# Audio-WestlakeU/FullSubNet

Measured on NVIDIA H100. Metric: frames_per_sec, higher is better.
Workload: dtype f16x3(hi+lo split, fp32-class)xf32acc

## Files before the change

### fullsubnet_b200/csrc/fsn_subband_tc.cu

```cuda
#include <cuda_fp16.h>
#include <stdlib.h>
#include <string.h>

#include "fsn_internal.cuh"
#include "fsn_tc_ptx.cuh"
#include "fsn_wgmma.cuh"

namespace fsn {
namespace tc {

using namespace ptx;

constexpr int NB = 32;
constexpr int KB = 64;
constexpr int KS = 32;
constexpr int US = 64;
constexpr int W_SUB = US * KS * 2;
constexpr int W_TILE = 4 * W_SUB;
constexpr int S_KBLK = NB * KB * 2;
constexpr int X_BLK = NB * KS * 2;
constexpr int MAX_STAGES = 4;
constexpr int MAX_MT = 3;
constexpr int OUT_T = 8;
constexpr int NTHREADS = 128 + 128 * MAX_MT;

struct PackedLayout {
  int H, MT, nkb0, nkb1, parts;
  size_t tiles0, tiles1;
  size_t off_bias, off_fcw, off_fcb, bytes;
};

__host__ __device__ inline PackedLayout packed_layout(int H, bool x3) {
  PackedLayout L;
  L.H = H; L.MT = H / 128;
  L.nkb0 = 1 + H / KS; L.nkb1 = 2 * H / KS;
  L.parts = x3 ? 2 : 1;
  L.tiles0 = (size_t)L.MT * L.nkb0 * L.parts;
  L.tiles1 = (size_t)L.MT * L.nkb1 * L.parts;
  L.off_bias = 2 * (L.tiles0 + L.tiles1) * W_TILE;
  L.off_fcw = L.off_bias + (size_t)2 * 4 * H * sizeof(float);
  L.off_fcb = L.off_fcw + (size_t)2 * H * sizeof(float);
  L.bytes = L.off_fcb + 256;
  return L;
}

__global__ void pack_kernel(const float* __restrict__ wih0, const float* __restrict__ whh0,
                            const float* __restrict__ wih1, const float* __restrict__ whh1,
                            const float* __restrict__ bih0, const float* __restrict__ bhh0,
                            const float* __restrict__ bih1, const float* __restrict__ bhh1,
                            const float* __restrict__ fcw, const float* __restrict__ fcb, int H, int Ksb, int x3,
                            int fc_out, uint8_t* __restrict__ out) {
  const PackedLayout L = packed_layout(H, x3 != 0);
  const size_t per_half = L.tiles0 + L.tiles1;
  const size_t total = 2 * per_half * 4 * US * 4;
  for (size_t i = blockIdx.x * (size_t)blockDim.x + threadIdx.x; i < total; i += (size_t)gridDim.x * blockDim.x) {
    const int c = (int)(i & 3);
    const int r = (int)((i >> 2) & (US - 1));
    const int g = (int)((i >> 8) & 3);
    const size_t st_abs = i >> 10;
    const int half = (int)(st_abs / per_half);
    size_t st = st_abs - half * per_half;
    const int layer = st >= L.tiles0;
    if (layer) st -= L.tiles0;
    const int part = (int)(st % L.parts);
    st /= L.parts;
    const int nkb = layer ? L.nkb1 : L.nkb0;
    const int kb = (int)(st % nkb);
    const int m = (int)(st / nkb);
    const int wrow = g * H + (half * L.MT + m) * US + r;
    __half v[8];
#pragma unroll
    for (int e = 0; e < 8; ++e) {
      const int kk = c * 8 + e;
      float w = 0.f;
      if (layer == 0) {
        if (kb == 0) { if (kk < Ksb) w = wih0[(size_t)wrow * Ksb + kk]; }
        else w = whh0[(size_t)wrow * H + (kb - 1) * KS + kk];
      } else {
        const int k = kb * KS + kk;
        w = (k < H) ? wih1[(size_t)wrow * H + k] : whh1[(size_t)wrow * H + (k - H)];
      }
      const __half hi = __float2half_rn(w);
      v[e] = part ? __float2half_rn(w - __half2float(hi)) : hi;
    }
    uint8_t* dst = out + st_abs * W_TILE + g * W_SUB + swz64_off(r, c * 8);
    *reinterpret_cast<uint4*>(dst) = *reinterpret_cast<const uint4*>(v);
  }
  float* bias = reinterpret_cast<float*>(out + L.off_bias);
  float* pfcw = reinterpret_cast<float*>(out + L.off_fcw);
  float* pfcb = reinterpret_cast<float*>(out + L.off_fcb);
  for (int i = blockIdx.x * blockDim.x + threadIdx.x; i < 4 * H; i += gridDim.x * blockDim.x) {
    bias[i] = bih0[i] + bhh0[i];
    bias[4 * H + i] = bih1[i] + bhh1[i];
  }
  for (int i = blockIdx.x * blockDim.x + threadIdx.x; i < 2 * H; i += gridDim.x * blockDim.x)
    pfcw[i] = (i < fc_out * H) ? fcw[i] : 0.f;
  if (blockIdx.x == 0 && threadIdx.x < 2) pfcb[threadIdx.x] = ((int)threadIdx.x < fc_out) ? fcb[threadIdx.x] : 0.f;
}

struct Smem {
  uint32_t w, x, h0, h1, lo, fcw, fcp, outst, rows, bars, total;
};
__host__ __device__ inline Smem smem_plan(int H, int stages, bool x3) {
  Smem s;
  const int nkh = H / KB;
  uint32_t o = 0;
  s.w = o; o += stages * W_TILE;
  s.x = o; o += 2 * X_BLK;
  s.h0 = o; o += 2 * nkh * S_KBLK;
  s.h1 = o; o += nkh * S_KBLK;
  s.lo = o; o += x3 ? (o - s.x) : 0;
  s.fcw = o; o += 4 * MAX_MT * 2 * NB * 4;
  s.fcp = o; o += 2 * 2 * NB * 4;
  s.outst = o; o += NB * 2 * OUT_T * 4;
  s.rows = o; o += NB * 16;
  s.bars = o; o += 256;
  s.total = o;
  return s;
}

struct Bars {
  uint64_t w_full[MAX_STAGES], w_empty[MAX_STAGES];
  uint64_t x_full[2], x_empty[2];
  uint64_t h0_ready[2], h0_empty[2];
  uint64_t h1_ready, h1_empty, fc_done;
  uint64_t l1_done;
  uint64_t fcp_full[2], fcp_empty[2];
  uint64_t turn[MAX_MT];
};
static_assert(sizeof(Bars) <= 256, "barrier block too large");

struct RowInfo {
  int src_b, src_f;
  float scale;
  int out_idx;
};

struct KArgs {
  const uint8_t* packed;
  const float* magT; const float* fbT; const float* inv2;
  const float* unit_scale;
  float* crm;
  int R, F, Tp, la, T, Ns, Nf, H, Ksb, act, Fsub, stages, cluster;
  int src_T, shrink;
  RowMap map;
  long long* stamps;
  int stamp_ctas, stamp_its;
};

enum ProbeField {
  PF_T_BEGIN = 0,
  PF_T_MMA0 = 1,
  PF_T_MMA1 = 2,
  PF_T_END = 3,
  PF_OPERAND = 4,
  PF_TURN = 5,
  PF_W_FULL = 6,
  PF_WAIT_GROUP = 7,
  PF_GROUP_LAT = 8,
  PF_STAGES = 9,
  PF_CELL = 10,
  PF_L1_DONE = 11,
  PF_H1_EMPTY = 12,
  PF_H0_EMPTY = 13,
  PF_FC_DONE = 14,
  PF_GT_BEGIN = 15,
  PROBE_FIELDS = 16
};
constexpr int PROBE_SLOTS = MAX_MT + 1;
static_assert(PROBE_FIELDS == FSN_SB_PROBE_FIELDS && PROBE_SLOTS == FSN_SB_PROBE_SLOTS,
              "probe record layout differs from fsn_b200.h (and fullsubnet_b200/_lib.py)");

__device__ __forceinline__ long long globaltimer() {
  uint64_t t;
  asm volatile("mov.u64 %0, %%globaltimer;" : "=l"(t));
  return (long long)t;
}

__device__ __forceinline__ float act_apply(float v, int act) {
  switch (act) {
    case FSN_ACT_RELU: return fmaxf(v, 0.f);
    case FSN_ACT_TANH: return tanhf(v);
    case FSN_ACT_RELU6: return fminf(fmaxf(v, 0.f), 6.f);
    default: return v;
  }
}
template <bool X3> __device__ __forceinline__ float sg(float x) { return X3 ? 1.0f / (1.0f + expf(-x)) : fast_sigmoid(x); }
template <bool X3> __device__ __forceinline__ float th(float x) { return X3 ? 1.0f - 2.0f / (1.0f + expf(2.0f * x)) : fast_tanh(x); }

__device__ __forceinline__ void release_stage(uint32_t bar, uint32_t pred, uint32_t local, uint32_t remote,
                                              uint32_t rank) {
  mbar_arrive_elect_if(bar, pred & local);
  mbar_arrive_remote_elect_if(bar, rank, pred & remote);
}

template <bool X3, bool PROBE>
__global__ void __launch_bounds__(NTHREADS, 1) sb_lstm_tc_kernel(const __grid_constant__ KArgs a) {
  constexpr int PARTS = X3 ? 2 : 1;
  long long pt = 0;
  auto mark = [&]() -> uint32_t {
    if constexpr (PROBE) {
      const long long n = clock64();
      const uint32_t d = (uint32_t)(n - pt);
      pt = n;
      return d;
    } else {
      return 0u;
    }
  };
  auto record = [&](int it, int layer, int slot) -> long long* {
    return a.stamps + ((((size_t)blockIdx.x * a.stamp_its + it) * 2 + layer) * PROBE_SLOTS + slot) * PROBE_FIELDS;
  };
  const bool probe_cta = PROBE && (int)blockIdx.x < a.stamp_ctas;
  extern __shared__ uint8_t smem_raw[];
  uint8_t* smem = smem_raw + ((1024u - (smem_u32(smem_raw) & 1023u)) & 1023u);
  const int H = a.H;
  const int MT = H / 128;
  const int nkh = H / KB;
  const int STAGES = a.stages;
  const int CL = a.cluster;
  const uint32_t cl_rank = cluster_ctarank();
  const int half = (int)(cl_rank & 1u);
  const uint32_t peer = cl_rank ^ 1u;
  const uint16_t cl_mask = (uint16_t)((0x55u & ((1u << (2 * CL)) - 1u)) << half);
  const Smem sp = smem_plan(H, STAGES, X3);
  const uint32_t LO = sp.lo - sp.x;
  const PackedLayout PL = packed_layout(H, X3);
  Bars& bars = *reinterpret_cast<Bars*>(smem + sp.bars);
  RowInfo* rows = reinterpret_cast<RowInfo*>(smem + sp.rows);
  float* fc_part = reinterpret_cast<float*>(smem + sp.fcw);
  float* fcp = reinterpret_cast<float*>(smem + sp.fcp);
  float* outst = reinterpret_cast<float*>(smem + sp.outst);
  const int warp = threadIdx.x >> 5, lane = threadIdx.x & 31;
  const int row0 = (blockIdx.x >> 1) * NB;
  const int Tp = a.Tp;

  if (threadIdx.x == 0) {
    for (int s = 0; s < STAGES; ++s) { mbar_init(&bars.w_full[s], 1); mbar_init(&bars.w_empty[s], CL); }
    for (int i = 0; i < 2; ++i) {
      mbar_init(&bars.x_full[i], 1); mbar_init(&bars.x_empty[i], 4 * MT);
      mbar_init(&bars.h0_ready[i], 5 * MT);
      mbar_init(&bars.h0_empty[i], MT);
      mbar_init(&bars.fcp_full[i], 1); mbar_init(&bars.fcp_empty[i], 1);
    }
    mbar_init(&bars.h1_ready, 5 * MT);
    mbar_init(&bars.h1_empty, MT);
    mbar_init(&bars.fc_done, 1);
    mbar_init(&bars.l1_done, 4 * MT);
    for (int m = 0; m < MAX_MT; ++m) mbar_init(&bars.turn[m], 4);
    asm volatile("fence.mbarrier_init.release.cluster;" ::: "memory");
  }
  if (threadIdx.x < NB) {
    RowInfo ri;
    const int r = row0 + threadIdx.x;
    ri.src_b = -1; ri.src_f = 0; ri.scale = 0.f; ri.out_idx = 0;
    if (r < a.R) {
      row_to_unit(a.map, r, ri.src_b, ri.src_f);
      ri.scale = a.inv2[ri.src_b];
      const int bq = r / a.Fsub, fq = r - bq * a.Fsub;
      ri.out_idx = bq * 2 * a.Fsub + fq;
    }
    rows[threadIdx.x] = ri;
  }
  {
    uint4* z = reinterpret_cast<uint4*>(smem + sp.x);
    const int n16 = (sp.fcw - sp.x) / 16;
    for (int i = threadIdx.x; i < n16; i += blockDim.x) z[i] = make_uint4(0, 0, 0, 0);
  }
  fence_proxy_async_smem();
  __syncthreads();
  cluster_sync_all();

  if (warp < 4) {
    asm volatile("setmaxnreg.dec.sync.aligned.u32 56;");
  if (warp == 0) {
    const uint8_t* stream = a.packed + (size_t)half * (PL.tiles0 + PL.tiles1) * W_TILE;
    uint32_t stage = 0, phase = 0;
    for (int it = 0; it <= Tp; ++it) {
      const size_t t_begin = (it < Tp) ? 0 : PL.tiles0;
      const size_t t_end = (it >= 1) ? PL.tiles0 + PL.tiles1 : PL.tiles0;
      const uint8_t* src = stream + t_begin * W_TILE;
      long long p_t0 = 0, p_g0 = 0;
      uint32_t p_empty = 0;
      if constexpr (PROBE) { p_g0 = globaltimer(); p_t0 = clock64(); pt = p_t0; }
      for (size_t tile = t_begin; tile < t_end; ++tile, src += W_TILE) {
        mark();
        mbar_wait_cta<false>(&bars.w_empty[stage], phase ^ 1);
        p_empty += mark();
        if (elect_one()) {
          mbar_expect_tx(&bars.w_full[stage], W_TILE);
          if (CL == 1) {
            bulk_g2s(smem + sp.w + stage * W_TILE, src, W_TILE, &bars.w_full[stage]);
          } else {
            const uint32_t slice = W_TILE / CL, off = (cl_rank >> 1) * slice;
            bulk_g2s_mc(smem + sp.w + stage * W_TILE + off, src + off, slice, &bars.w_full[stage], cl_mask);
          }
        }
        __syncwarp();
        if (++stage == (uint32_t)STAGES) { stage = 0; phase ^= 1; }
      }
      if (probe_cta && it < a.stamp_its && lane == 0) {
        long long* r = record(it, 0, MAX_MT);
        r[PF_T_BEGIN] = p_t0; r[PF_T_END] = clock64(); r[PF_OPERAND] = p_empty;
        r[PF_STAGES] = (long long)(t_end - t_begin); r[PF_GT_BEGIN] = p_g0;
      }
    }
  } else if (warp == 2) {
    const int nmag = 2 * a.Ns + 1;
    for (int t = 0; t < Tp; ++t) {
      mbar_wait_cta<true>(&bars.x_empty[t & 1], ((t >> 1) & 1) ^ 1);
      uint8_t* xb = smem + sp.x + (t & 1) * X_BLK;
      int f0 = t, f1 = t + 1;
      if (a.shrink > 1 && t > 0) { f0 = 1 + (t - 1) * a.shrink; f1 = min(f0 + a.shrink, a.src_T); }
      const float wmean = 1.0f / (float)(f1 - f0);
#pragma unroll 4
      for (int n = 0; n < NB; ++n) {
        const RowInfo ri = rows[n];
        float v = 0.f;
        if (ri.src_b >= 0 && lane < a.Ksb) {
          const int col = (lane < nmag) ? reflect_idx(ri.src_f + lane - a.Ns, a.F)
                                        : reflect_idx(ri.src_f + (lane - nmag) - a.Nf, a.F);
          const float* src = (lane < nmag) ? a.magT : a.fbT;
          if (a.shrink <= 1) {
            v = src[((size_t)ri.src_b * a.src_T + t) * a.F + col];
            v *= a.unit_scale ? a.unit_scale[(size_t)t * a.R + row0 + n] : ri.scale;
          } else {
            for (int fr = f0; fr < f1; ++fr) v += src[((size_t)ri.src_b * a.src_T + fr) * a.F + col];
            v *= wmean * (a.unit_scale ? a.unit_scale[(size_t)t * a.R + row0 + n] : ri.scale);
          }
        }
        const __half hi = __float2half_rn(v);
        *reinterpret_cast<__half*>(xb + swz64_off(n, lane)) = hi;
        if (X3) *reinterpret_cast<__half*>(xb + LO + swz64_off(n, lane)) = __float2half_rn(v - __half2float(hi));
      }
      fence_proxy_async_smem();
      __syncwarp();
      if (lane == 0) mbar_arrive(&bars.x_full[t & 1]);
    }
  } else if (warp == 3) {
    const float fcb0 = half ? 0.f : reinterpret_cast<const float*>(a.packed + PL.off_fcb)[0];
    const float fcb1 = half ? 0.f : reinterpret_cast<const float*>(a.packed + PL.off_fcb)[1];
    const RowInfo ri = rows[lane];
    int staged = 0, t_stage0 = 0;
    for (int t = 0; t < Tp; ++t) {
      mbar_wait_cta<true>(&bars.h1_ready, t & 1);
      float s0 = fcb0, s1 = fcb1;
      if (t >= a.la) {
        for (int w = 0; w < 4 * MT; ++w) {
          s0 += fc_part[(w * 2 + 0) * NB + lane];
          s1 += fc_part[(w * 2 + 1) * NB + lane];
        }
      }
      __syncwarp();
      if (lane == 0) mbar_arrive(&bars.fc_done);
      if (t < a.la) continue;
      const int u = t - a.la, b = u & 1;
      float* pb = fcp + b * 2 * NB;
      if (half) {
        mbar_wait<true>(&bars.fcp_empty[b], ((u >> 1) & 1) ^ 1);
        st_remote_f32(pb + lane, peer, s0);
        st_remote_f32(pb + NB + lane, peer, s1);
        __syncwarp();
        if (lane == 0) mbar_arrive_cluster(&bars.fcp_full[b], peer);
        continue;
      }
      mbar_wait<true>(&bars.fcp_full[b], (u >> 1) & 1);
      s0 += pb[lane];
      s1 += pb[NB + lane];
      __syncwarp();
      if (lane == 0) mbar_arrive_cluster(&bars.fcp_empty[b], peer);
      if (staged == 0) t_stage0 = u;
      outst[(lane * 2 + 0) * OUT_T + staged] = act_apply(s0, a.act);
      outst[(lane * 2 + 1) * OUT_T + staged] = act_apply(s1, a.act);
      ++staged;
      if (staged == OUT_T || t == Tp - 1) {
        if (ri.src_b >= 0) {
#pragma unroll
          for (int o = 0; o < 2; ++o) {
            float* dst = a.crm + ((size_t)ri.out_idx + (size_t)o * a.Fsub) * a.T + t_stage0;
            for (int i = 0; i < staged; ++i) dst[i] = outst[(lane * 2 + o) * OUT_T + i];
          }
        }
        staged = 0;
      }
    }
  }
  } else {
    asm volatile("setmaxnreg.inc.sync.aligned.u32 152;");
    const int m = __shfl_sync(0xffffffffu, (warp - 4) >> 2, 0);
    const int q = __shfl_sync(0xffffffffu, warp & 3, 0);
    const int s = half * MT + m;
    if (m < MT) {
      const float* bias_g = reinterpret_cast<const float*>(a.packed + PL.off_bias);
      const float* fcw = reinterpret_cast<const float*>(a.packed + PL.off_fcw);
      float* my_part = fc_part + (size_t)(warp - 4) * 2 * NB;
      float c0[16], c1[16];
#pragma unroll
      for (int i = 0; i < 16; ++i) c0[i] = c1[i] = 0.f;
      const uint32_t a_lo0 = wg::desc_lo(smem_u32(smem + sp.w));
      const uint32_t w_full0 = smem_u32(&bars.w_full[0]), w_empty0 = smem_u32(&bars.w_empty[0]);
      const uint32_t turn_next = smem_u32(&bars.turn[m + 1 < MT ? m + 1 : 0]);
      const uint32_t rel_local = CL == 1 && q == 0, rel_remote = CL > 1 && q < CL;
      const uint32_t rel_rank = 2 * q + half;
      int h0_seen = 0, h1_seen = 0, turns = 0;
      bool first_block = true;
      size_t tile_base = 0;
      for (int it = 0; it <= Tp; ++it) {
        for (int layer = 0; layer < 2; ++layer) {
          const int t = it - layer;
          if (t < 0 || t >= Tp) continue;
          long long p_t0 = 0, p_g0 = 0, p_mma0 = 0, p_mma1 = 0, p_commit = 0, p_commit_prev = 0;
          uint32_t p_opnd = 0, p_turn = 0, p_wfull = 0, p_wgw = 0, p_lat = 0, p_cell = 0, p_l1 = 0, p_h1e = 0, p_h0e = 0,
                   p_fc = 0;
          if constexpr (PROBE) { p_g0 = globaltimer(); p_t0 = clock64(); pt = p_t0; }
          if (layer == 0) {
            mbar_wait_cta<false>(&bars.x_full[t & 1], (t >> 1) & 1);
            for (; h0_seen < t; ++h0_seen) mbar_wait_cta<false>(&bars.h0_ready[h0_seen & 1], (h0_seen >> 1) & 1);
          } else {
            for (; h0_seen < t + 1; ++h0_seen) mbar_wait_cta<false>(&bars.h0_ready[h0_seen & 1], (h0_seen >> 1) & 1);
            for (; h1_seen < t; ++h1_seen) mbar_wait_cta<false>(&bars.h1_ready, h1_seen & 1);
          }
          p_opnd += mark();
          const uint32_t x_addr = smem_u32(smem + sp.x + (t & 1) * X_BLK);
          const uint32_t h0_cur = smem_u32(smem + sp.h0 + (t & 1) * nkh * S_KBLK);
          const uint32_t h0_prev = smem_u32(smem + sp.h0 + ((t + 1) & 1) * nkh * S_KBLK);
          const uint32_t h1_prev = smem_u32(smem + sp.h1);
          const int nkb = layer ? PL.nkb1 : PL.nkb0;
          const size_t first = tile_base + (layer ? ((it < Tp) ? PL.tiles0 : 0) : 0) + (size_t)m * nkb * PARTS;
          float acc[4][16];
#pragma unroll
          for (int g = 0; g < 4; ++g) {
#pragma unroll
            for (int i = 0; i < 16; ++i) acc[g][i] = 0.f;
            wg::fence_operand(acc[g]);
          }
          int prev_stage = -1;
          if (m > 0 || !first_block) { mbar_wait_cta<false>(&bars.turn[m], turns & 1); ++turns; }
          first_block = false;
          p_turn += mark();
          p_mma0 = pt;
          int stage = __shfl_sync(0xffffffffu, (int)(first % (size_t)STAGES), 0);
          uint32_t wphase = __shfl_sync(0xffffffffu, (uint32_t)((first / (size_t)STAGES) & 1), 0);
          auto issue_stage = [&](int part, uint32_t bd, uint32_t b_hi, uint32_t ends_block) {
            mark();
            mbar_wait_cta_warp(w_full0 + 8 * stage, wphase);
            p_wfull += mark();
            mbar_arrive_elect_if(turn_next, ends_block);
            wg::fence();
            const uint32_t ad = a_lo0 + stage * (W_TILE >> 4);
#pragma unroll
            for (int kk = 0; kk < 2; ++kk)
#pragma unroll
              for (int g = 0; g < 4; ++g) {
                const uint32_t a_off = g * (W_SUB >> 4) + kk * 2;
                wg::mma_f16_n32_w(acc[g], ad, a_off, wg::DESC_SW64_HI, bd, kk * 2, b_hi);
                if (X3 && part == 0) wg::mma_f16_n32_w(acc[g], ad, a_off, wg::DESC_SW64_HI, bd, (LO >> 4) + kk * 2, b_hi);
              }
            wg::commit();
            if constexpr (PROBE) p_commit = clock64();
            mark();
            wg::wait<1>();
            p_wgw += mark();
            if constexpr (PROBE) {
              if (prev_stage >= 0) p_lat += (uint32_t)(pt - p_commit_prev);
              p_commit_prev = p_commit;
            }
            release_stage(w_empty0 + 8 * prev_stage, prev_stage >= 0, rel_local, rel_remote, rel_rank);
            prev_stage = stage;
            if (++stage == STAGES) { stage = 0; wphase ^= 1; }
          };
          if (layer == 0) {
#pragma unroll
            for (int part = 0; part < PARTS; ++part) issue_stage(part, wg::desc_lo(x_addr), wg::DESC_SW64_HI, 0u);
          }
          const int nseg = layer ? 2 : 1;
          int seg = 0;
          do {
            uint32_t bd = wg::desc_lo(layer == 0 ? h0_prev : seg == 0 ? h0_cur : h1_prev);
            int kb = 0;
            do {
              const uint32_t ends_block = seg == nseg - 1 && kb == nkh - 1;
#pragma unroll
              for (int part = 0; part < PARTS; ++part) issue_stage(part, bd, wg::DESC_SW128_HI, 0u);
#pragma unroll
              for (int part = 0; part < PARTS; ++part)
                issue_stage(part, bd + (64 >> 4), wg::DESC_SW128_HI, part == PARTS - 1 ? ends_block : 0u);
              bd += S_KBLK >> 4;
            } while (++kb < nkh);
          } while (++seg < nseg);
          mark();
          wg::wait<0>();
#pragma unroll
          for (int g = 0; g < 4; ++g) wg::fence_operand(acc[g]);
          p_wgw += mark();
          if constexpr (PROBE) { p_lat += (uint32_t)(pt - p_commit_prev); p_mma1 = pt; }
          release_stage(w_empty0 + 8 * prev_stage, 1u, rel_local, rel_remote, rel_rank);
          if (lane == 0) mbar_arrive(layer ? &bars.l1_done : &bars.x_empty[t & 1]);
          if (layer == 1 && lane == 0) {
            if (q == 2) mbar_arrive_remote(&bars.h0_empty[t & 1], peer);
            if (q == 3) mbar_arrive_remote(&bars.h1_empty, peer);
          }
          p_cell += mark();
          if (layer == 1 && t >= 1) mbar_wait_cta<false>(&bars.fc_done, (t - 1) & 1);
          p_fc += mark();
          float fsum[2][8];
#pragma unroll
          for (int i = 0; i < 16; ++i) fsum[i >> 3][i & 7] = 0.f;
          __half hv[2][8];
          __half lv[2][8];
          uint8_t* hb = smem + (layer ? sp.h1 : sp.h0 + (t & 1) * nkh * S_KBLK) + s * S_KBLK;
#pragma unroll
          for (int hh = 0; hh < 2; ++hh) {
            const int u = s * US + 16 * q + (lane >> 2) + 8 * hh;
            const float* bl = bias_g + (layer ? 4 * H : 0);
            const float bi = bl[u], bff = bl[H + u], bg = bl[2 * H + u], bo = bl[3 * H + u];
            const float w0 = fcw[u], w1 = fcw[H + u];
#pragma unroll
            for (int j = 0; j < 4; ++j)
#pragma unroll
              for (int e = 0; e < 2; ++e) {
                const int ri = 4 * j + 2 * hh + e;
                const int ci = hh * 8 + j * 2 + e;
                const float cp = layer ? c1[ci] : c0[ci];
                const float cn = sg<X3>(acc[1][ri] + bff) * cp + sg<X3>(acc[0][ri] + bi) * th<X3>(acc[2][ri] + bg);
                if (layer) c1[ci] = cn; else c0[ci] = cn;
                const float h = sg<X3>(acc[3][ri] + bo) * th<X3>(cn);
                const __half hi = __float2half_rn(h);
                hv[hh][j * 2 + e] = hi;
                lv[hh][j * 2 + e] = __float2half_rn(h - __half2float(hi));
                if (layer) { fsum[0][j * 2 + e] += h * w0; fsum[1][j * 2 + e] += h * w1; }
              }
          }
          if (layer == 1) {
#pragma unroll
            for (int o = 0; o < 2; ++o)
#pragma unroll
              for (int r = 0; r < 8; ++r) {
                float v = fsum[o][r];
                v += __shfl_xor_sync(0xffffffffu, v, 4);
                v += __shfl_xor_sync(0xffffffffu, v, 8);
                v += __shfl_xor_sync(0xffffffffu, v, 16);
                fsum[o][r] = v;
              }
            if (lane < 4) {
#pragma unroll
              for (int o = 0; o < 2; ++o)
#pragma unroll
                for (int r = 0; r < 8; ++r) my_part[o * NB + 8 * (r >> 1) + 2 * lane + (r & 1)] = fsum[o][r];
            }
            p_cell += mark();
            mbar_wait_cta<false>(&bars.l1_done, t & 1);
            p_l1 += mark();
            mbar_wait_cta<false>(&bars.h1_empty, t & 1);
            p_h1e += mark();
          } else if (t >= 2) {
            p_cell += mark();
            mbar_wait_cta<false>(&bars.h0_empty[t & 1], ((t - 2) >> 1) & 1);
            p_h0e += mark();
          }
#pragma unroll
          for (int hh = 0; hh < 2; ++hh) {
            const int u = 16 * q + (lane >> 2) + 8 * hh;
            uint8_t* ub = hb + (u & 7) * 2;
            const int chunk = u >> 3;
#pragma unroll
            for (int j = 0; j < 4; ++j)
#pragma unroll
              for (int e = 0; e < 2; ++e) {
                const int n = 8 * j + 2 * (lane & 3) + e;
                uint8_t* p = ub + (n >> 3) * 1024 + (n & 7) * 128 + ((chunk ^ (n & 7)) << 4);
                *reinterpret_cast<__half*>(p) = hv[hh][j * 2 + e];
                if (X3) *reinterpret_cast<__half*>(p + LO) = lv[hh][j * 2 + e];
              }
          }
          fence_proxy_async_smem();
          __syncwarp();
          uint64_t* ready = layer ? &bars.h1_ready : &bars.h0_ready[t & 1];
          if (lane == 0) mbar_arrive(ready);
          named_sync(1 + m, 128);
          if (q == 0 && lane == 0) {
            mbar_arrive_expect_tx_remote(ready, peer, PARTS * S_KBLK);
            bulk_s2s_remote(hb, S_KBLK, ready, peer);
            if (X3) bulk_s2s_remote(hb + LO, S_KBLK, ready, peer);
          }
          if constexpr (PROBE) {
            p_cell += mark();
            if (probe_cta && it < a.stamp_its && q == 0 && lane == 0) {
              long long* r = record(it, layer, m);
              r[PF_T_BEGIN] = p_t0; r[PF_T_MMA0] = p_mma0; r[PF_T_MMA1] = p_mma1; r[PF_T_END] = pt;
              r[PF_OPERAND] = p_opnd; r[PF_TURN] = p_turn; r[PF_W_FULL] = p_wfull; r[PF_WAIT_GROUP] = p_wgw;
              r[PF_GROUP_LAT] = p_lat; r[PF_STAGES] = nkb * PARTS; r[PF_CELL] = p_cell; r[PF_L1_DONE] = p_l1;
              r[PF_H1_EMPTY] = p_h1e; r[PF_H0_EMPTY] = p_h0e; r[PF_FC_DONE] = p_fc; r[PF_GT_BEGIN] = p_g0;
            }
          }
        }
        tile_base += ((it < Tp) ? PL.tiles0 : 0) + ((it >= 1) ? PL.tiles1 : 0);
      }
    }
  }

  __syncthreads();
  cluster_sync_all();
}

}

static int sb_ksb(const fsn_model_desc* d) { return (2 * d->sb_num_neighbors + 1) + (2 * d->fb_num_neighbors + 1); }

static bool sb_tc_shape_ok(int H, int Ksb) { return H % 128 == 0 && H / 128 <= tc::MAX_MT && H >= 128 && Ksb <= tc::KS; }

bool sb_tc_supported(const fsn_model_desc* d) {
  if (d->cell_type != FSN_CELL_LSTM) return false;
  return sb_tc_shape_ok(d->sb_hidden, sb_ksb(d));
}

size_t sb_tc_packed_bytes_raw(int H, bool x3) { return tc::packed_layout(H, x3).bytes; }

size_t sb_tc_packed_bytes(const fsn_model_desc* d) {
  if (!sb_tc_supported(d)) return 0;
  return sb_tc_packed_bytes_raw(d->sb_hidden, d->precision == FSN_PREC_F16X3_TC);
}

int sb_tc_pack_raw(const fsn_seq_weights* sb, int H, int Ksb, int fc_out, void* packed, cudaStream_t st, bool x3) {
  FSN_REQUIRE(sb_tc_shape_ok(H, Ksb), FSN_ERR_UNSUPPORTED,
              "the fp16 tensor-core LSTM stack needs a hidden size in {128,256,384} and an input width <= 32");
  int dev = 0, sms = 132;
  cudaGetDevice(&dev);
  cudaDeviceGetAttribute(&sms, cudaDevAttrMultiProcessorCount, dev);
  tc::pack_kernel<<<sms * 4, 256, 0, st>>>(sb->w_ih[0], sb->w_hh[0], sb->w_ih[1], sb->w_hh[1], sb->b_ih[0], sb->b_hh[0],
                                           sb->b_ih[1], sb->b_hh[1], sb->fc_w, sb->fc_b, H, Ksb, x3 ? 1 : 0, fc_out,
                                           (uint8_t*)packed);
  FSN_CHECK_LAUNCH("sb pack_kernel");
  return FSN_OK;
}

int sb_tc_pack(const fsn_model_desc* d, const fsn_seq_weights* sb, void* packed, cudaStream_t st) {
  FSN_REQUIRE(sb_tc_supported(d), FSN_ERR_UNSUPPORTED,
              "FSN_PREC_F16_TC / FSN_PREC_F16X3_TC need sb_hidden in {128,256,384} and sub-band input width <= 32");
  return sb_tc_pack_raw(sb, d->sb_hidden, sb_ksb(d), 2, packed, st, d->precision == FSN_PREC_F16X3_TC);
}

template <bool X3, bool PROBE = false>
static int sb_tc_config(int H, int stages, int cluster, int pairs, cudaStream_t st, cudaLaunchConfig_t& cfg,
                        cudaLaunchAttribute* attr) {
  const tc::Smem sp = tc::smem_plan(H, stages, X3);
  const size_t smem = sp.total + 1024;
  int rc = check_cuda(cudaFuncSetAttribute(tc::sb_lstm_tc_kernel<X3, PROBE>, cudaFuncAttributeMaxDynamicSharedMemorySize,
                                           (int)smem), "sb_lstm_tc smem attr");
  if (rc) return rc;
  memset(&cfg, 0, sizeof(cfg));
  cfg.gridDim = dim3(2 * pairs);
  cfg.blockDim = dim3(128 + 128 * (H / 128));
  cfg.dynamicSmemBytes = smem;
  cfg.stream = st;
  attr[0].id = cudaLaunchAttributeClusterDimension;
  attr[0].val.clusterDim.x = 2 * cluster;
  attr[0].val.clusterDim.y = 1;
  attr[0].val.clusterDim.z = 1;
  cfg.attrs = attr;
  cfg.numAttrs = 1;
  return FSN_OK;
}

template <bool X3, bool PROBE>
static int sb_tc_launch(const tc::KArgs& a, int H, cudaStream_t st) {
  const int pairs = cdiv(cdiv(a.R, tc::NB), a.cluster) * a.cluster;
  cudaLaunchConfig_t cfg;
  cudaLaunchAttribute attr[1];
  int rc = sb_tc_config<X3, PROBE>(H, a.stages, a.cluster, pairs, st, cfg, attr);
  if (rc) return rc;
  rc = check_cuda(cudaLaunchKernelEx(&cfg, tc::sb_lstm_tc_kernel<X3, PROBE>, a), "sb_lstm_tc_kernel launch");
  if (rc) return rc;
  FSN_CHECK_LAUNCH("sb_lstm_tc_kernel");
  return FSN_OK;
}

int sb_tc_forward(const SbTcArgs& s, cudaStream_t st) {
  tc::KArgs a;
  a.packed = (const uint8_t*)s.packed;
  a.magT = s.magT; a.fbT = s.fbT; a.inv2 = s.inv2; a.unit_scale = s.unit_scale; a.crm = s.crm;
  a.R = s.map.B * s.map.Fsub; a.F = s.F; a.Tp = s.steps > 0 ? s.steps : s.Tp; a.la = s.la; a.T = a.Tp - s.la;
  a.src_T = s.Tp; a.shrink = s.shrink > 1 ? s.shrink : 1;
  a.Ns = s.Ns; a.Nf = s.Nf; a.H = s.H; a.Ksb = (2 * s.Ns + 1) + (2 * s.Nf + 1); a.act = s.act;
  a.Fsub = s.map.Fsub; a.map = s.map;
  a.stamps = s.stamps; a.stamp_ctas = s.stamp_ctas; a.stamp_its = s.stamp_its;
  FSN_REQUIRE(sb_tc_shape_ok(a.H, a.Ksb), FSN_ERR_UNSUPPORTED, "sb_lstm_tc: unsupported hidden size %d / input width %d",
              a.H, a.Ksb);
  static int stages_env = -1;
  if (stages_env < 0) {
    const char* e = getenv("FSN_TC_STAGES");
    stages_env = e ? atoi(e) : 4;
    if (stages_env < 2) stages_env = 2;
    if (stages_env > tc::MAX_STAGES) stages_env = tc::MAX_STAGES;
  }
  static int cluster_env = -1;
  if (cluster_env < 0) {
    const char* e = getenv("FSN_TC_CLUSTER");
    cluster_env = e ? atoi(e) : 1;
    if (cluster_env != 1 && cluster_env != 2 && cluster_env != 4) cluster_env = 1;
  }
  a.stages = s.stages ? s.stages : stages_env;
  a.cluster = s.cluster ? s.cluster : cluster_env;
  if (s.stamps) return s.x3 ? sb_tc_launch<true, true>(a, s.H, st) : sb_tc_launch<false, true>(a, s.H, st);
  return s.x3 ? sb_tc_launch<true, false>(a, s.H, st) : sb_tc_launch<false, false>(a, s.H, st);
}

}

extern "C" size_t fsn_debug_sb_lstm_tc_packed_bytes(int H, int x3) {
  return fsn::sb_tc_shape_ok(H, 0) ? fsn::sb_tc_packed_bytes_raw(H, x3 != 0) : 0;
}

extern "C" int fsn_debug_sb_lstm_tc_max_clusters(int H, int x3, int stages, int cluster, int* clusters) {
  using namespace fsn;
  FSN_REQUIRE(cluster == 1 || cluster == 2 || cluster == 4, FSN_ERR_UNSUPPORTED,
              "sb_lstm_tc: cluster size %d (1, 2 or 4)", cluster);
  FSN_REQUIRE(stages >= 2 && stages <= tc::MAX_STAGES, FSN_ERR_UNSUPPORTED, "sb_lstm_tc: ring depth %d (2, 3 or 4)",
              stages);
  FSN_REQUIRE(sb_tc_shape_ok(H, 0), FSN_ERR_UNSUPPORTED, "sb_lstm_tc: unsupported hidden size %d", H);
  FSN_REQUIRE(clusters, FSN_ERR_SHAPE, "sb_lstm_tc: missing output");
  cudaLaunchConfig_t cfg;
  cudaLaunchAttribute attr[1];
  int rc = x3 ? sb_tc_config<true>(H, stages, cluster, cluster, nullptr, cfg, attr)
              : sb_tc_config<false>(H, stages, cluster, cluster, nullptr, cfg, attr);
  if (rc) return rc;
  return x3 ? check_cuda(cudaOccupancyMaxActiveClusters(clusters, tc::sb_lstm_tc_kernel<true, false>, &cfg), "sb_lstm_tc occupancy")
            : check_cuda(cudaOccupancyMaxActiveClusters(clusters, tc::sb_lstm_tc_kernel<false, false>, &cfg), "sb_lstm_tc occupancy");
}

static int sb_lstm_tc_hook(const fsn_seq_weights* sb, int H, int Ns, int Nf, int fc_out, int act, int x3,
                           const float* magT, const float* fbT, int B, int F, int src_T, int G, const float* inv2,
                           const float* unit_scale, int la, int steps, int shrink, int stages, int cluster, void* packed,
                           float* crm, long long* stamps, int stamp_ctas, int stamp_steps, fsn_stream_t stream) {
  using namespace fsn;
  FSN_REQUIRE(cluster == 0 || cluster == 1 || cluster == 2 || cluster == 4, FSN_ERR_UNSUPPORTED,
              "sb_lstm_tc: cluster size %d (0, 1, 2 or 4)", cluster);
  FSN_REQUIRE(stages == 0 || (stages >= 2 && stages <= tc::MAX_STAGES), FSN_ERR_UNSUPPORTED,
              "sb_lstm_tc: ring depth %d (0, 2, 3 or 4)", stages);
  FSN_REQUIRE(sb && magT && fbT && inv2 && packed && crm, FSN_ERR_SHAPE, "sb_lstm_tc: missing buffer");
  FSN_REQUIRE(B > 0 && F > 1 && src_T > 0 && Ns >= 0 && Nf >= 0 && Ns < F && Nf < F, FSN_ERR_SHAPE,
              "sb_lstm_tc: bad shape B=%d F=%d src_T=%d Ns=%d Nf=%d", B, F, src_T, Ns, Nf);
  FSN_REQUIRE(fc_out == 1 || fc_out == 2, FSN_ERR_SHAPE, "sb_lstm_tc: fc_out %d (1 or 2)", fc_out);
  FSN_REQUIRE(act >= FSN_ACT_NONE && act <= FSN_ACT_RELU6, FSN_ERR_SHAPE, "sb_lstm_tc: activation %d", act);
  FSN_REQUIRE(shrink >= 1 && G >= 1, FSN_ERR_SHAPE, "sb_lstm_tc: shrink %d / groups %d", shrink, G);
  const int g = (B > 1 && G > 1) ? G : 1;
  FSN_REQUIRE(B == 1 || B > G, FSN_ERR_SHAPE, "sb_lstm_tc: batch size %d <= num_groups %d", B, G);
  const int Fsub = g > 1 ? F / g : F;
  FSN_REQUIRE(Fsub > 0, FSN_ERR_SHAPE, "sb_lstm_tc: num_freqs < num_groups");
  const int max_steps = shrink > 1 ? 1 + cdiv(src_T - 1, shrink) : src_T;
  FSN_REQUIRE(steps > 0 && steps <= max_steps && la >= 0 && la < steps, FSN_ERR_SHAPE,
              "sb_lstm_tc: steps %d / look-ahead %d for %d source frames (shrink %d)", steps, la, src_T, shrink);
  FSN_REQUIRE(!(unit_scale && shrink > 1), FSN_ERR_UNSUPPORTED, "sb_lstm_tc: per-step scales with time down-sampling");
  FSN_REQUIRE(sb_tc_shape_ok(H, (2 * Ns + 1) + (2 * Nf + 1)), FSN_ERR_UNSUPPORTED,
              "sb_lstm_tc: unsupported hidden size %d / input width %d", H, (2 * Ns + 1) + (2 * Nf + 1));
  if (stamps) {
    const int ctas = 2 * cdiv(B * Fsub, tc::NB);
    FSN_REQUIRE(stamp_ctas >= 1 && stamp_ctas <= ctas, FSN_ERR_SHAPE, "sb_lstm_tc probe: %d sampled CTAs (1 .. %d)",
                stamp_ctas, ctas);
    FSN_REQUIRE(stamp_steps >= 1 && stamp_steps <= steps + 1, FSN_ERR_SHAPE,
                "sb_lstm_tc probe: %d sampled iterations (1 .. steps + 1 = %d)", stamp_steps, steps + 1);
  }
  cudaStream_t st = (cudaStream_t)stream;
  int rc = sb_tc_pack_raw(sb, H, (2 * Ns + 1) + (2 * Nf + 1), fc_out, packed, st, x3 != 0);
  if (rc) return rc;
  SbTcArgs a;
  memset(&a, 0, sizeof(a));
  a.packed = packed; a.magT = magT; a.fbT = fbT; a.inv2 = inv2; a.unit_scale = unit_scale; a.crm = crm;
  a.B = B; a.F = F; a.Tp = src_T; a.la = la; a.Ns = Ns; a.Nf = Nf; a.H = H; a.act = act;
  a.steps = steps; a.shrink = shrink; a.x3 = x3 != 0;
  a.map = RowMap{B, F, Fsub, g};
  a.stages = stages; a.cluster = cluster;
  a.stamps = stamps; a.stamp_ctas = stamp_ctas; a.stamp_its = stamp_steps;
  return sb_tc_forward(a, st);
}

extern "C" int fsn_debug_sb_lstm_tc(const fsn_seq_weights* sb, int H, int Ns, int Nf, int fc_out, int act, int x3,
                                    const float* magT, const float* fbT, int B, int F, int src_T, int G,
                                    const float* inv2, const float* unit_scale, int la, int steps, int shrink, int stages,
                                    int cluster, void* packed, float* crm, fsn_stream_t stream) {
  return sb_lstm_tc_hook(sb, H, Ns, Nf, fc_out, act, x3, magT, fbT, B, F, src_T, G, inv2, unit_scale, la, steps, shrink,
                         stages, cluster, packed, crm, nullptr, 0, 0, stream);
}

extern "C" int fsn_debug_sb_lstm_tc_probe(const fsn_seq_weights* sb, int H, int Ns, int Nf, int fc_out, int act, int x3,
                                          const float* magT, const float* fbT, int B, int F, int src_T, int G,
                                          const float* inv2, const float* unit_scale, int la, int steps, int shrink,
                                          int stages, int cluster, void* packed, float* crm, long long* stamps,
                                          int stamp_ctas, int stamp_steps, fsn_stream_t stream) {
  using namespace fsn;
  FSN_REQUIRE(stamps, FSN_ERR_SHAPE, "sb_lstm_tc probe: missing stamp buffer");
  return sb_lstm_tc_hook(sb, H, Ns, Nf, fc_out, act, x3, magT, fbT, B, F, src_T, G, inv2, unit_scale, la, steps, shrink,
                         stages, cluster, packed, crm, stamps, stamp_ctas, stamp_steps, stream);
}
```

Baseline: 127,500.

## Hand off weight-ring turn early using double-generation full barriers

Duplicates the w_full mbarrier set so consumers can tell apart two consecutive generations of the weight ring. The turn token now passes to the next M-tile warpgroup several K-blocks before the current block finishes, instead of at its last stage. The next consumer can then start waiting on and consuming tiles while the current one drains its tail, hiding handoff latency. The cost is more complex phase tracking, and a parity aliasing risk if the generation assumptions are off.

```diff
diff --git a/fullsubnet_b200/csrc/fsn_subband_tc.cu b/fullsubnet_b200/csrc/fsn_subband_tc.cu
--- a/fullsubnet_b200/csrc/fsn_subband_tc.cu
+++ b/fullsubnet_b200/csrc/fsn_subband_tc.cu
@@ -120,7 +120,7 @@
 }
 
 struct Bars {
-  uint64_t w_full[MAX_STAGES], w_empty[MAX_STAGES];
+  uint64_t w_full[2][MAX_STAGES], w_empty[MAX_STAGES];
   uint64_t x_full[2], x_empty[2];
   uint64_t h0_ready[2], h0_empty[2];
   uint64_t h1_ready, h1_empty, fc_done;
@@ -129,6 +129,7 @@
   uint64_t turn[MAX_MT];
 };
 static_assert(sizeof(Bars) <= 256, "barrier block too large");
+static_assert(1 + 256 / KS >= 2 * MAX_STAGES, "a block of MT >= 2 must span two ring generations (turn[])");
 
 struct RowInfo {
   int src_b, src_f;
@@ -236,7 +237,9 @@
   const int Tp = a.Tp;
 
   if (threadIdx.x == 0) {
-    for (int s = 0; s < STAGES; ++s) { mbar_init(&bars.w_full[s], 1); mbar_init(&bars.w_empty[s], CL); }
+    for (int s = 0; s < STAGES; ++s) {
+      mbar_init(&bars.w_full[0][s], 1); mbar_init(&bars.w_full[1][s], 1); mbar_init(&bars.w_empty[s], CL);
+    }
     for (int i = 0; i < 2; ++i) {
       mbar_init(&bars.x_full[i], 1); mbar_init(&bars.x_empty[i], 4 * MT);
       mbar_init(&bars.h0_ready[i], 5 * MT);
@@ -288,12 +291,13 @@
         mbar_wait_cta<false>(&bars.w_empty[stage], phase ^ 1);
         p_empty += mark();
         if (elect_one()) {
-          mbar_expect_tx(&bars.w_full[stage], W_TILE);
+          uint64_t* full = &bars.w_full[phase][stage];
+          mbar_expect_tx(full, W_TILE);
           if (CL == 1) {
-            bulk_g2s(smem + sp.w + stage * W_TILE, src, W_TILE, &bars.w_full[stage]);
+            bulk_g2s(smem + sp.w + stage * W_TILE, src, W_TILE, full);
           } else {
             const uint32_t slice = W_TILE / CL, off = (cl_rank >> 1) * slice;
-            bulk_g2s_mc(smem + sp.w + stage * W_TILE + off, src + off, slice, &bars.w_full[stage], cl_mask);
+            bulk_g2s_mc(smem + sp.w + stage * W_TILE + off, src + off, slice, full, cl_mask);
           }
         }
         __syncwarp();
@@ -398,8 +402,9 @@
 #pragma unroll
       for (int i = 0; i < 16; ++i) c0[i] = c1[i] = 0.f;
       const uint32_t a_lo0 = wg::desc_lo(smem_u32(smem + sp.w));
-      const uint32_t w_full0 = smem_u32(&bars.w_full[0]), w_empty0 = smem_u32(&bars.w_empty[0]);
+      const uint32_t w_full0 = smem_u32(&bars.w_full[0][0]), w_empty0 = smem_u32(&bars.w_empty[0]);
       const uint32_t turn_next = smem_u32(&bars.turn[m + 1 < MT ? m + 1 : 0]);
+      const int turn_kb = nkh - min(nkh, STAGES / PARTS);
       const uint32_t rel_local = CL == 1 && q == 0, rel_remote = CL > 1 && q < CL;
       const uint32_t rel_rank = 2 * q + half;
       int h0_seen = 0, h1_seen = 0, turns = 0;
@@ -440,12 +445,13 @@
           p_turn += mark();
           p_mma0 = pt;
           int stage = __shfl_sync(0xffffffffu, (int)(first % (size_t)STAGES), 0);
-          uint32_t wphase = __shfl_sync(0xffffffffu, (uint32_t)((first / (size_t)STAGES) & 1), 0);
-          auto issue_stage = [&](int part, uint32_t bd, uint32_t b_hi, uint32_t ends_block) {
+          uint32_t wset = __shfl_sync(0xffffffffu, (uint32_t)((first / (size_t)STAGES) & 1), 0);
+          uint32_t wphase = __shfl_sync(0xffffffffu, (uint32_t)((first / (size_t)STAGES / 2) & 1), 0);
+          auto issue_stage = [&](int part, uint32_t bd, uint32_t b_hi, uint32_t hand_on) {
             mark();
-            mbar_wait_cta_warp(w_full0 + 8 * stage, wphase);
+            mbar_wait_cta_warp(w_full0 + wset * (8 * MAX_STAGES) + 8 * stage, wphase);
             p_wfull += mark();
-            mbar_arrive_elect_if(turn_next, ends_block);
+            mbar_arrive_elect_if(turn_next, hand_on);
             wg::fence();
             const uint32_t ad = a_lo0 + stage * (W_TILE >> 4);
 #pragma unroll
@@ -467,7 +473,7 @@
             }
             release_stage(w_empty0 + 8 * prev_stage, prev_stage >= 0, rel_local, rel_remote, rel_rank);
             prev_stage = stage;
-            if (++stage == STAGES) { stage = 0; wphase ^= 1; }
+            if (++stage == STAGES) { stage = 0; wphase ^= wset; wset ^= 1; }
           };
           if (layer == 0) {
 #pragma unroll
@@ -478,13 +484,13 @@
           do {
             uint32_t bd = wg::desc_lo(layer == 0 ? h0_prev : seg == 0 ? h0_cur : h1_prev);
             int kb = 0;
+#pragma unroll 1
             do {
-              const uint32_t ends_block = seg == nseg - 1 && kb == nkh - 1;
-#pragma unroll
-              for (int part = 0; part < PARTS; ++part) issue_stage(part, bd, wg::DESC_SW128_HI, 0u);
-#pragma unroll
-              for (int part = 0; part < PARTS; ++part)
-                issue_stage(part, bd + (64 >> 4), wg::DESC_SW128_HI, part == PARTS - 1 ? ends_block : 0u);
+              const uint32_t hand_on = seg == nseg - 1 && kb == turn_kb;
+#pragma unroll
+              for (int part = 0; part < PARTS; ++part) issue_stage(part, bd, wg::DESC_SW128_HI, part == 0 ? hand_on : 0u);
+#pragma unroll
+              for (int part = 0; part < PARTS; ++part) issue_stage(part, bd + (64 >> 4), wg::DESC_SW128_HI, 0u);
               bd += S_KBLK >> 4;
             } while (++kb < nkh);
           } while (++seg < nseg);
```

After: 127,300, median of 6. Within noise of the previous version (-0.2%).
